# shihchinw/rlShaders

Hardware: AMD Instinct MI355X
Metric: BSDF Gsamples/sec (eval+sample+pdf) (higher is better)
Workload: dtype f32

## Files before the change

__graft_entry__.py:

```python
from __future__ import annotations

import os
import subprocess
import sys
from pathlib import Path

ROOT = Path(__file__).resolve().parent
REF_SRC_DEFAULT = "/root/reference"
for p in (str(ROOT), str(ROOT / "tests")):
    if p not in sys.path:
        sys.path.insert(0, p)


def build() -> None:
    from rlshaders_amd import build as b
    lib = b.build_library(verbose=False)
    assert lib.exists(), lib
    b.build_host_examples()
    b.build_trace_example()
    p = subprocess.run(["make", "-C", str(ROOT / "oracle")], capture_output=True, text=True)
    if p.returncode != 0:
        raise RuntimeError(f"oracle build failed:\n{p.stdout}\n{p.stderr}")
    ref_src = Path(os.environ.get("RLS_REF_SRC", REF_SRC_DEFAULT))
    if (ref_src / "src" / "rlGgx.h").exists():
        p = subprocess.run(["make", "-C", str(ROOT / "oracle"), "ref", f"REF_SRC={ref_src}"], capture_output=True,
                           text=True)
        if p.returncode != 0:
            raise RuntimeError(f"reference build failed:\n{p.stdout}\n{p.stderr}")
    import rlshaders_amd
    rlshaders_amd.load()
    from rlshaders_amd import trace
    trace.load()


def smoke() -> None:
    import numpy as np
    import torch

    import cases
    import oracle_lib as O
    import rlshaders_amd as R
    from gpu_util import dev, ggx_oracle, ggx_sampler, host

    assert torch.cuda.is_available(), "smoke() needs a GPU"
    ctx = R.Context(0)
    n = 1 << 14
    c = cases.ggx_mixed(cases.SEED_PARITY, n)
    x = cases.xi(cases.SEED_PARITY, n, 4)
    s = ggx_sampler(ctx, c)
    out = [host(t) for t in s.reflectRefract(dev(x[0]), dev(x[1]), dev(x[2]), dev(x[3]))]
    ref = ggx_oracle(O, c).reflect_refract(x[0], x[1], x[2], x[3])
    names = ("wi", "f", "pdf", "fresnel", "wt", "weight")
    for name, a, b in zip(names, out, ref):
        st = cases.summarize(cases.rel_err(a, b))
        print(f"smoke {name}: median {st['median']:.2e} p99.9 {st['p999']:.2e} frac>1e-5 {st['frac_gt_1e5']:.2e}")
        assert st["nonfinite"] == 0 and st["max"] <= 1e-5, (name, st)
    f = host(s.evalBrdf(dev(ref[0])))
    assert cases.summarize(cases.rel_err(f, ref[1]))["max"] <= 1e-5
    ctx.close()
    print("smoke ok")


if __name__ == "__main__":
    build()
    if len(sys.argv) > 1 and sys.argv[1] == "smoke":
        smoke()
```

rlshaders_amd/build.py:

```python
from __future__ import annotations

import os
import shutil
import subprocess
import sys
from concurrent.futures import ThreadPoolExecutor
from pathlib import Path

PKG = Path(__file__).resolve().parent
CSRC = PKG / "csrc"
LIBDIR = PKG / "lib"
OBJDIR = PKG / "build"
LIB = LIBDIR / "librlshaders_amd.so"
ARCH = "gfx950"

SOURCES = ["shade.hip", "integrate.hip", "lights.hip", "scatter.hip", "skin.hip", "ggx.hip", "disney.hip", "sss.hip", "alternates.hip", "context.hip", "pipeline.hip",
           "libm_check.hip"]
FAST_UNITS = {"ggx.hip", "disney.hip", "sss.hip", "skin.hip", "integrate.hip", "lights.hip", "scatter.hip", "shade.hip", "alternates.hip"}
HEADERS = [CSRC / "rls_device.hpp", CSRC / "rls_libm.hpp", CSRC / "rls_libm_tables.inc", CSRC / "rls_libm_flavour_args.inc", CSRC / "rls_internal.hpp", CSRC / "rls_loops.hpp",
           PKG.parent / "include" / "rlshaders_amd.h", PKG.parent / "include" / "rlshaders_amd_diag.h"]

HIPCC_FLAGS = [
    f"--offload-arch={ARCH}", "-O3", "-std=c++17", "-fPIC",
    "-ffp-contract=off", "-fno-fast-math",
# ... 42 lines not shown
    def run(cmd):
        if verbose:
            print(" ".join(cmd), flush=True)
        p = subprocess.run(cmd, capture_output=True, text=True)
        if p.returncode != 0:
            raise RuntimeError(f"hipcc failed:\n{' '.join(cmd)}\n{p.stdout}\n{p.stderr}")
        return p

    if jobs:
        with ThreadPoolExecutor(max_workers=min(4, len(jobs))) as ex:
            list(ex.map(run, jobs))
    if force or jobs or _stale(lib, objs):
        run([hipcc, f"--offload-arch={ARCH}", "-shared", "-fPIC", "-o", str(lib), *map(str, objs)])
    return lib


TRACE_CSRC = PKG / "csrc_trace"
TRACE_SOURCES = ["trace.hip"]
TRACE_LIB = LIBDIR / "librls_trace.so"
TRACE_HEADERS = [*sorted(TRACE_CSRC.glob("*.hpp")), PKG.parent / "include" / "rlshaders_amd_trace.h"]


def build_trace_library(force: bool = False, verbose: bool = False) -> Path:
    hipcc = _hipcc()
    main = build_library(verbose=verbose)
    objdir = OBJDIR / "trace"
    objdir.mkdir(parents=True, exist_ok=True)
    jobs, objs = [], []
    for name in TRACE_SOURCES:
        src = TRACE_CSRC / name
        for suffix, flag in (("", "RLS_FAST=0"), ("_fast", "RLS_FAST=1")):
            obj = objdir / (src.stem + suffix + ".o")
            objs.append(obj)
            if force or _stale(obj, [src, *HEADERS, *TRACE_HEADERS, Path(__file__)]):
                jobs.append([hipcc, *HIPCC_FLAGS, f"-cuid=rls_trace.{src.stem}{suffix}", f"-D{flag}", "-c", str(src),
                             "-o", str(obj)])

    def run(cmd):
        if verbose:
            print(" ".join(cmd), flush=True)
        p = subprocess.run(cmd, capture_output=True, text=True)
        if p.returncode != 0:
            raise RuntimeError(f"hipcc failed:\n{' '.join(cmd)}\n{p.stdout}\n{p.stderr}")

    if jobs:
        with ThreadPoolExecutor(max_workers=min(4, len(jobs))) as ex:
            list(ex.map(run, jobs))
    if force or jobs or _stale(TRACE_LIB, [*objs, main]):
        run([hipcc, f"--offload-arch={ARCH}", "-shared", "-fPIC", "-o", str(TRACE_LIB), *map(str, objs),
             f"-L{LIBDIR}", "-lrlshaders_amd", "-Wl,-rpath,$ORIGIN"])
    return TRACE_LIB


def build_trace_example(verbose: bool = False) -> Path:
    OBJDIR.mkdir(exist_ok=True)
    lib = build_trace_library(verbose=verbose)
    src, out = PKG / "host" / "example_trace.cpp", OBJDIR / "example_trace"
    if _stale(out, [src, PKG / "host" / "rls_trace.hpp", lib, LIB, *HEADERS, *TRACE_HEADERS]):
        cmd = ["g++", "-std=c++14", "-O2", "-Wall", f"-I{PKG.parent / 'include'}", f"-I{PKG / 'host'}", str(src), "-o", str(out),
               f"-L{LIBDIR}", "-lrls_trace", "-lrlshaders_amd", f"-Wl,-rpath,{LIBDIR}", "-L/opt/rocm/lib", "-Wl,-rpath,/opt/rocm/lib"]
        if verbose:
            print(" ".join(cmd), flush=True)
        p = subprocess.run(cmd, capture_output=True, text=True)
        if p.returncode != 0:
            raise RuntimeError(f"host example example_trace failed to build:\n{p.stdout}\n{p.stderr}")
    return out


def build_host_examples(verbose: bool = False) -> Path:
    OBJDIR.mkdir(exist_ok=True)
    first = OBJDIR / "example_arnold_stub"
    for name in ("example_arnold_stub", "example_multi_gpu", "example_host_pipeline", "test_arnold_stub"):
        src = PKG / "host" / f"{name}.cpp"
        out = OBJDIR / name
        if not src.exists():
            continue
        if _stale(out, [src, PKG / "host" / "rls_batch.hpp", PKG / "host" / "rl_arnold_stub.hpp", LIB, *HEADERS]):
            cmd = ["g++", "-std=c++14", "-O2", "-Wall", "-pthread", f"-I{PKG.parent / 'include'}", f"-I{PKG / 'host'}",
                   str(src), "-o", str(out), f"-L{LIBDIR}", "-lrlshaders_amd", f"-Wl,-rpath,{LIBDIR}",
                   "-L/opt/rocm/lib", "-Wl,-rpath,/opt/rocm/lib"]
            if verbose:
                print(" ".join(cmd), flush=True)
            p = subprocess.run(cmd, capture_output=True, text=True)
            if p.returncode != 0:
                raise RuntimeError(f"host example {name} failed to build:\n{p.stdout}\n{p.stderr}")
    return first


if __name__ == "__main__":
    args = sys.argv[1:]
    variant = args[args.index("--variant") + 1] if "--variant" in args else ""
    defines = [a[2:] for a in args if a.startswith("-D")]
    extra = []
    for i, a in enumerate(args):
        if a.startswith(("-f", "-m", "-O")):
            extra.append(a)
            if a == "-mllvm":
                extra.append(args[i + 1])
    print(build_library(force="--force" in args, verbose=True, variant=variant, defines=defines, extra=extra))
```

rlshaders_amd/codeid.py:

```python
from __future__ import annotations

import hashlib
import re
import struct
from functools import lru_cache
from pathlib import Path
from typing import Dict, List, Optional, Tuple

BUNDLE_MAGIC = b"__CLANG_OFFLOAD_BUNDLE__"
KERNEL_ID_SCHEME = 2
HASHED_SECTIONS = (".text", ".rodata", ".data")


def _sections(elf: bytes) -> Dict[str, Tuple[int, int, int]]:
    if elf[:4] != b"\x7fELF" or elf[4] != 2 or elf[5] != 1:
        raise ValueError("not a little-endian ELF64 image")
    shoff, = struct.unpack_from("<Q", elf, 0x28)
    shentsize, shnum, shstrndx = struct.unpack_from("<HHH", elf, 0x3A)
    heads = []
    for k in range(shnum):
        name, typ, _flags, _addr, off, size = struct.unpack_from("<IIQQQQ", elf, shoff + k * shentsize)
        heads.append((name, typ, off, size))
    _, _, stroff, strsize = heads[shstrndx]
    strtab = elf[stroff:stroff + strsize]
# ... 172 lines not shown
        h.update(name.encode() + b"\0" + struct.pack("<Q", size) + bytes(body))
    return h.hexdigest()[:16], [s[0] for s in syms if s[1] == 2]


def mangled_fragment(kernel: str) -> Optional[str]:
    m = re.search(r"([A-Za-z_][A-Za-z0-9_]*)\s*<([^<>]*)>\s*(?:\(|$)", kernel.strip())
    if not m:
        m = re.search(r"([A-Za-z_][A-Za-z0-9_]*)\s*(?:\(|$)", kernel.strip())
        return f"{len(m.group(1))}{m.group(1)}" if m else None
    name, args = m.group(1), [a.strip() for a in m.group(2).split(",") if a.strip()]
    enc = ""
    for a in args:
        if not re.fullmatch(r"-?\d+", a):
            return None
        enc += f"Li{'n' + a[1:] if a.startswith('-') else a}E"
    return f"{len(name)}{name}I{enc}E"


class DeviceCode:

    def __init__(self, path):
        self.path = str(path)
        objs = code_objects(fatbin(path))
        self.units = [unit_digest(e) for e in objs]
        self.kernels: Dict[str, str] = {}
        for e in objs:
            self.kernels.update(kernel_digests(e))
        self.library_id = hashlib.sha256("\n".join(sorted(u for u, _ in self.units)).encode()).hexdigest()[:16]

    def unit_of_kernel(self, kernel: str) -> Optional[str]:
        frag = mangled_fragment(kernel)
        if not frag:
            return None
        hits = sorted({u for u, syms in self.units if any(frag in s for s in syms)})
        return hits[0] if len(hits) == 1 else None

    def kernel_id(self, kernel: str) -> Optional[str]:
        frag = mangled_fragment(kernel)
        if not frag:
            return None
        hits = sorted({k for name, k in self.kernels.items() if frag in name})
        return hits[0] if len(hits) == 1 else None

    def record(self, kernel: Optional[str] = None) -> dict:
        rec = {"library_id": self.library_id}
        if kernel:
            rec["kernel"] = kernel
            rec["unit_id"] = self.unit_of_kernel(kernel)
            rec["kernel_id"] = self.kernel_id(kernel)
            rec["kernel_id_scheme"] = KERNEL_ID_SCHEME
        return rec


@lru_cache(maxsize=8)
def _cached(path: str, mtime: float, size: int) -> DeviceCode:
    return DeviceCode(path)


def device_code(path) -> DeviceCode:
    p = Path(path).resolve()
    st = p.stat()
    return _cached(str(p), st.st_mtime, st.st_size)


if __name__ == "__main__":
    import json
    import sys
    args = sys.argv[1:]
    lib = args[0] if args and args[0].endswith((".so", ".o")) or (args and ".so." in args[0]) else None
    if lib is None:
        from rlshaders_amd.build import LIB
        lib, names = LIB, args
    else:
        names = args[1:]
    dc = DeviceCode(lib)
    out = {"library": str(lib), "library_id": dc.library_id, "units": len(dc.units)}
    if names:
        out["kernels"] = {k: {"unit_id": dc.unit_of_kernel(k), "kernel_id": dc.kernel_id(k)} for k in names}
    else:
        out["unit_ids"] = sorted(u for u, _ in dc.units)
    print(json.dumps(out, indent=1))
```

rlshaders_amd/csrc/context.hip:

```cpp
#include <stdarg.h>
#include <stdlib.h>
#include <string.h>

#include "rls_internal.hpp"

namespace {
thread_local char g_error[512] = "";
}

namespace rlsh {

void set_error(const char *fmt, ...)
{
    va_list ap;
    va_start(ap, fmt);
    vsnprintf(g_error, sizeof(g_error), fmt, ap);
    va_end(ap);
}

rls_status hip_fail(hipError_t e, const char *what)
{
    set_error("HIP error %d (%s) in %s", (int)e, hipGetErrorString(e), what);
    (void)hipGetLastError();
    return e == hipErrorOutOfMemory ? RLS_ERR_OUT_OF_MEMORY : RLS_ERR_HIP;
}

}

using namespace rlsd;

extern "C" {

const char *rls_last_error(void) { return g_error; }

const char *rls_status_string(rls_status s)
{
    switch (s) {
    case RLS_OK: return "ok";
    case RLS_ERR_INVALID_ARGUMENT: return "invalid argument";
    case RLS_ERR_NO_DEVICE: return "no HIP device";
    case RLS_ERR_HIP: return "HIP runtime error";
    case RLS_ERR_OUT_OF_MEMORY: return "out of device memory";
    case RLS_ERR_UNSUPPORTED: return "unsupported";
    case RLS_ERR_ABORTED: return "stopped by a callback";
    default: return "unknown status";
    }
}

int rls_version(void) { return RLS_VERSION_MAJOR * 1000 + RLS_VERSION_MINOR; }

rls_status rls_context_create(int device_ordinal, rls_context **out)
{
    RLS_REQUIRE(out != nullptr, "out is NULL");
    *out = nullptr;
    int count = 0;
    hipError_t e = hipGetDeviceCount(&count);
    if (e != hipSuccess || count <= 0) {
        rlsh::set_error("rls_context_create: no HIP device visible (%s)",
                        e == hipSuccess ? "count = 0" : hipGetErrorString(e));
        return RLS_ERR_NO_DEVICE;
    }
    if (device_ordinal < 0 || device_ordinal >= count) {
        rlsh::set_error("rls_context_create: device %d out of range [0, %d)", device_ordinal, count);
        return RLS_ERR_NO_DEVICE;
    }
    RLS_HIP_TRY(hipSetDevice(device_ordinal));
    hipDeviceProp_t prop;
    RLS_HIP_TRY(hipGetDeviceProperties(&prop, device_ordinal));

    rls_context *ctx = (rls_context *)calloc(1, sizeof(rls_context));
    if (!ctx) { rlsh::set_error("rls_context_create: host allocation failed"); return RLS_ERR_OUT_OF_MEMORY; }
    ctx->device = device_ordinal;
    ctx->compute_units = prop.multiProcessorCount > 0 ? prop.multiProcessorCount : 256;
    ctx->blocks_per_cu = 64;
    if (const char *s = getenv("RLS_BLOCKS_PER_CU")) {
        int v = atoi(s);
        if (v >= 1 && v <= 4096) ctx->blocks_per_cu = v;
    }
    hipError_t e1 = hipStreamCreateWithFlags(&ctx->own_stream, hipStreamNonBlocking);
    hipError_t e2 = e1 == hipSuccess ? hipEventCreate(&ctx->ev_start) : e1;
    hipError_t e3 = e2 == hipSuccess ? hipEventCreate(&ctx->ev_stop) : e2;
    if (e3 == hipSuccess) e3 = hipEventCreate(&ctx->ev_probe_start);
    if (e3 == hipSuccess) e3 = hipEventCreate(&ctx->ev_probe_stop);
    hipError_t e4 = e3 == hipSuccess ? hipMalloc((void **)&ctx->scratch_u64, sizeof(unsigned long long)) : e3;
    if (e4 != hipSuccess) {
        rls_status st = rlsh::hip_fail(e4, "rls_context_create");
        rls_context_destroy(ctx);
        return st;
    }
    ctx->stream = ctx->own_stream;
    *out = ctx;
    return RLS_OK;
}

void rls_context_destroy(rls_context *ctx)
{
    if (!ctx) return;
    (void)hipSetDevice(ctx->device);
    if (ctx->capturing) {
        hipGraph_t g = nullptr;
        if (hipStreamEndCapture(ctx->stream, &g) == hipSuccess && g) (void)hipGraphDestroy(g);
        (void)hipGetLastError();
    }
    if (ctx->own_stream) (void)hipStreamSynchronize(ctx->own_stream);
    if (ctx->scratch_u64) (void)hipFree(ctx->scratch_u64);
    if (ctx->stamp_buf) (void)hipFree(ctx->stamp_buf);
    if (ctx->ev_start) (void)hipEventDestroy(ctx->ev_start);
    if (ctx->ev_stop) (void)hipEventDestroy(ctx->ev_stop);
    if (ctx->ev_probe_start) (void)hipEventDestroy(ctx->ev_probe_start);
    if (ctx->ev_probe_stop) (void)hipEventDestroy(ctx->ev_probe_stop);
    if (ctx->own_stream) (void)hipStreamDestroy(ctx->own_stream);
    free(ctx);
}

int rls_device_count(void)
{
    int n = 0;
    if (hipGetDeviceCount(&n) != hipSuccess) { (void)hipGetLastError(); return 0; }
    return n;
}

rls_status rls_shard_range(int64_t total, int rank, int world, int64_t *first, int64_t *count)
{
    RLS_REQUIRE(first != nullptr && count != nullptr, "NULL argument");
    RLS_REQUIRE(world >= 1 && rank >= 0 && rank < world && total >= 0, "bad shard request");
    const __int128 lo = (__int128)total * rank / world, hi = (__int128)total * (rank + 1) / world;
    *first = (int64_t)lo;
    *count = (int64_t)(hi - lo);
    return RLS_OK;
}

rls_status rls_context_set_stream(rls_context *ctx, void *hip_stream)
{
    RLS_REQUIRE(ctx != nullptr, "ctx is NULL");
    RLS_REQUIRE(!ctx->capturing, "not allowed while a launch graph is being recorded");
    ctx->stream = (hipStream_t)hip_stream;
    return RLS_OK;
}

rls_status rls_context_use_own_stream(rls_context *ctx)
{
    RLS_REQUIRE(ctx != nullptr, "ctx is NULL");
    RLS_REQUIRE(!ctx->capturing, "not allowed while a launch graph is being recorded");
// ... 514 lines not shown
```

rlshaders_amd/csrc/ggx.hip:

```cpp
#include "rls_internal.hpp"

using namespace rlsd;

namespace {

using namespace rlsh;

#define RLS_GGX_ARGS(a0) reload_args(a0)

enum { MIXED = 0, STREAMED_ALL = 1, UNIFORM_MATERIAL = 2 };

template <int MODE>
__device__ __forceinline__ Ggx load_closure(const rls_ggx_closure &c, Idx i, const GgxMaterial &um)
{
    constexpr bool STREAMED = MODE == STREAMED_ALL;
    V3 wo = ld3(c.wo, i), N = ld3(c.N, i), T = ld3(c.T, i);
    const PIndex<Idx> k = pindex<MODE == MIXED>(c.materials, i);
    float kr, kg, kb;
    ldrgb<STREAMED>(c.KsColor, k, kr, kg, kb);
    if (MODE == UNIFORM_MATERIAL)
        return ggx_from_material(um, wo, N, T, c.exiting ? (c.exiting[i.full()] != 0) : false, kr, kg, kb);
    float rough = ldp<STREAMED>(c.specularRoughness, k);
    float ior = ldp<STREAMED>(c.ior, k);
    float aniso = ldp<STREAMED>(c.anisotropic, k);
    bool exiting = c.exiting ? (c.exiting[i.full()] != 0) : false;
    return ggx_make(wo, N, T, exiting, kr, kg, kb, ior, rough, aniso);
}

#ifndef RLS_GGX_WAVES
#define RLS_GGX_WAVES(OP) ((OP) == OP_EVAL ? 6 : 8)
#endif
#define RLS_GGX_ATTR(OP) __launch_bounds__(rlsh::kBlock) __attribute__((amdgpu_waves_per_eu(RLS_GGX_WAVES(OP), RLS_GGX_WAVES(OP))))
template <int OP, int FAST_MATH, int MODE>
__device__ __forceinline__ void ggx_body(const GgxIO &a0)
{
    if (OP == OP_SAMPLE || OP == OP_FUSED || OP == OP_REFLECT_REFRACT || OP == OP_REFRACT || OP == OP_MICROFACET)
        stage_libm_tables();
    GgxMaterial um = {};
    if (MODE == UNIFORM_MATERIAL) {
        const rls_ggx_closure &c = a0.c;
        um = ggx_material_wave_uniform(ggx_material(c.ior.u, c.specularRoughness.u, c.anisotropic.u));
    }
    const TileRange tiles = tile_range(a0.n);
    for (int64_t base = tiles.first; base < tiles.end; base += tiles.step) {
        const Idx i = make_idx(base);
        if (i.full() >= a0.n) continue;
        const GgxIO a = RLS_GGX_ARGS(a0);
        Ggx g = load_closure<MODE>(a.c, i, um);

        if (OP == OP_SAMPLE || OP == OP_FUSED || OP == OP_REFLECT_REFRACT) {
            float rx = ldg(a.rx, i), ry = ldg(a.ry, i);
            VndfView w = vndf_view(g.view, g.fr, g.ax, g.ay);
            V3 M, M2;
            if (OP == OP_REFLECT_REFRACT) {
                float rx2 = ldg(a.rx2, i), ry2 = ldg(a.ry2, i);
                vndf_microfacet_pair(w, g.fr, rx, ry, w, g.fr, rx2, ry2, M, M2);
            } else {
                M = vndf_microfacet(w, g.fr, rx, ry);
            }
            V3 L = reflect_direction(g.view, M);
            float F = ggx_fresnel(g, L, M);
            {
                const GgxIO b = RLS_GGX_ARGS(a0);
                st3(b.wi, i, L);
                if (b.fresnel) stg(b.fresnel, i, F);
            }
            if (OP != OP_SAMPLE) {
                float fr, fg, fb, pdf;
                ggx_eval_pdf<true, true>(g, L, fr, fg, fb, pdf);
                const GgxIO b = RLS_GGX_ARGS(a0);
                strgb(b.f, i, fr, fg, fb);
                stg(b.pdf, i, pdf);
            }
            if (OP == OP_REFLECT_REFRACT) {
                V3 dir;
                ggx_refract(g, M2, dir);
                const float wgt = ggx_sample_weight(g, g.view, dir, M2);
                const GgxIO b = RLS_GGX_ARGS(a0);
                st3(b.wt, i, dir);
                stg(b.weight, i, wgt);
            }
// ... 3 lines not shown
            strgb(a.f, i, fr, fg, fb);
        } else if (OP == OP_PDF) {
            stg(a.pdf, i, ggx_pdf(g, ld3(a.cwi, i)));
        } else if (OP == OP_REFRACT) {
            float rx = ldg(a.rx, i), ry = ldg(a.ry, i);
            VndfView w = vndf_view(g.view, g.fr, g.ax, g.ay);
            V3 M = vndf_microfacet(w, g.fr, rx, ry);
            V3 dir;
            bool ok = ggx_refract(g, M, dir);
            st3(a.wt, i, dir);
            stg(a.weight, i, ggx_sample_weight(g, g.view, dir, M));
            if (a.refracted) a.refracted[i.full()] = ok ? 1 : 0;
        } else if (OP == OP_MICROFACET) {
            float rx = ldg(a.rx, i), ry = ldg(a.ry, i);
            V3 M;
            if (a.kernel == RLS_KERNEL_NDF) {
                M = ndf_microfacet(g, rx, ry);
            } else {
                VndfView w = vndf_view(g.view, g.fr, g.ax, g.ay);
                M = vndf_microfacet(w, g.fr, rx, ry);
            }
            st3(a.wi, i, M);
        } else if (OP == OP_NDF_PDF) {
            V3 H = normalize(g.view + ld3(a.cwi, i));
            stg(a.pdf, i, ndf_pdf(g, g.view, H));
        }
    }
}

template <int OP, int FAST_MATH, int MODE>
__global__ RLS_GGX_ATTR(OP) void ggx_kernel(GgxIO a0)
{
    ggx_body<OP, FAST_MATH, MODE>(a0);
}

#if RLS_DIAGNOSTICS
template <int OP, int FAST_MATH, int MODE>
__global__ RLS_GGX_ATTR(OP) void ggx_kernel_stamped(GgxIO a0, unsigned long long *stamps)
{
    ClockStamp<1> cs;
    cs.begin();
    ggx_body<OP, FAST_MATH, MODE>(a0);
    cs.end(stamps);
}
#endif

template <int OP>
rls_status launch_kernel(rls_context *ctx, const GgxIO &io, const char *name)
{
    const rls_ggx_closure &c = io.c;
    const bool streamed = !c.materials.id && c.KsColor.r && c.specularRoughness.v && c.ior.v && c.anisotropic.v;
    const bool uniform = !c.materials.id && !c.specularRoughness.v && !c.ior.v && !c.anisotropic.v;
    if constexpr (OP == OP_REFLECT_REFRACT)
        RLS_STAMPED_LAUNCH(streamed, (ggx_kernel_stamped<OP, RLS_FAST, STREAMED_ALL>),
                           rlsh::grid_for(ctx, io.n, rlsh::kBlock, RLS_CAP_MULT), io, name);
    if (streamed)
        hipLaunchKernelGGL((ggx_kernel<OP, RLS_FAST, STREAMED_ALL>), rlsh::grid_for(ctx, io.n, rlsh::kBlock, RLS_CAP_MULT), dim3(rlsh::kBlock), 0, ctx->stream, io);
    else if (uniform)
        hipLaunchKernelGGL((ggx_kernel<OP, RLS_FAST, UNIFORM_MATERIAL>), rlsh::grid_for_hoisting(ctx, io.n), dim3(rlsh::kBlock), 0, ctx->stream, io);
    else
        hipLaunchKernelGGL((ggx_kernel<OP, RLS_FAST, MIXED>), rlsh::grid_for(ctx, io.n, rlsh::kBlock, RLS_CAP_MULT), dim3(rlsh::kBlock), 0, ctx->stream, io);
    return rlsh::check_launch(name, RLS_FAST);
}

rls_status launch_ggx(rls_context *ctx, int op, const GgxIO &io, const char *name)
{
    switch (op) {
    case OP_SAMPLE: return launch_kernel<OP_SAMPLE>(ctx, io, name);
    case OP_EVAL: return launch_kernel<OP_EVAL>(ctx, io, name);
    case OP_PDF: return launch_kernel<OP_PDF>(ctx, io, name);
    case OP_FUSED: return launch_kernel<OP_FUSED>(ctx, io, name);
    case OP_REFRACT: return launch_kernel<OP_REFRACT>(ctx, io, name);
    case OP_REFLECT_REFRACT: return launch_kernel<OP_REFLECT_REFRACT>(ctx, io, name);
    case OP_MICROFACET: return launch_kernel<OP_MICROFACET>(ctx, io, name);
    default: return launch_kernel<OP_NDF_PDF>(ctx, io, name);
    }
}

}

RLS_FLAVOURS(ggx, rlsh::GgxIO)

#if !RLS_FAST

extern "C" {

rls_status rls_ggx_sample(rls_context *ctx, int64_t n, const rls_ggx_closure *c,
                          const float *rx, const float *ry, rls_vec3 wi, float *fresnel)
{
    RLS_PROLOGUE();
    if (rls_status s = rlsh::check_closure(__func__, c)) return s;
    RLS_REQUIRE(rx && ry, "rx/ry is NULL");
    RLS_REQUIRE(rlsh::has3(wi), "wi plane is NULL");
    GgxIO io = {};
    io.c = *c; io.rx = rx; io.ry = ry; io.wi = wi; io.fresnel = fresnel; io.n = n;
    return dispatch_ggx(ctx, OP_SAMPLE, io, "rls_ggx_sample");
}

rls_status rls_ggx_eval(rls_context *ctx, int64_t n, const rls_ggx_closure *c, rls_cvec3 wi, rls_rgb f)
{
    RLS_PROLOGUE();
    if (rls_status s = rlsh::check_closure(__func__, c)) return s;
    RLS_REQUIRE(rlsh::has3(wi) && rlsh::has3(f), "wi/f plane is NULL");
    GgxIO io = {};
    io.c = *c; io.cwi = wi; io.f = f; io.n = n;
    return dispatch_ggx(ctx, OP_EVAL, io, "rls_ggx_eval");
}

rls_status rls_ggx_pdf(rls_context *ctx, int64_t n, const rls_ggx_closure *c, rls_cvec3 wi, float *pdf)
{
    RLS_PROLOGUE();
    if (rls_status s = rlsh::check_closure(__func__, c)) return s;
    RLS_REQUIRE(rlsh::has3(wi) && pdf, "wi/pdf is NULL");
    GgxIO io = {};
    io.c = *c; io.cwi = wi; io.pdf = pdf; io.n = n;
    return dispatch_ggx(ctx, OP_PDF, io, "rls_ggx_pdf");
}

rls_status rls_ggx_sample_eval_pdf(rls_context *ctx, int64_t n, const rls_ggx_closure *c,
                                   const float *rx, const float *ry,
                                   rls_vec3 wi, rls_rgb f, float *pdf, float *fresnel)
{
    RLS_PROLOGUE();
    if (rls_status s = rlsh::check_closure(__func__, c)) return s;
    RLS_REQUIRE(rx && ry, "rx/ry is NULL");
    RLS_REQUIRE(rlsh::has3(wi) && rlsh::has3(f) && pdf, "wi/f/pdf is NULL");
    GgxIO io = {};
    io.c = *c; io.rx = rx; io.ry = ry; io.wi = wi; io.f = f; io.pdf = pdf; io.fresnel = fresnel; io.n = n;
    return dispatch_ggx(ctx, OP_FUSED, io, "rls_ggx_sample_eval_pdf");
}

rls_status rls_ggx_refract_sample(rls_context *ctx, int64_t n, const rls_ggx_closure *c,
                                  const float *rx, const float *ry,
                                  rls_vec3 wt, float *weight, uint8_t *refracted)
{
    RLS_PROLOGUE();
// ... 51 lines not shown
```

rlshaders_amd/csrc/pipeline.hip:

```cpp
#include <stdlib.h>
#include <string.h>

#include "rls_internal.hpp"

namespace {

struct Slot {
    rls_context *ctx;
    float *block;
    float **in, **out;
};

template <class HostPtr>
hipError_t copy_planes(bool up, int planes, HostPtr const *host, float *const *dev, int64_t dev_stride, int64_t p0,
                       int64_t count, int64_t n, hipStream_t stream, bool &strided)
{
    hipError_t e = hipSuccess;
    const size_t row = (size_t)count * sizeof(float);
    for (int k = 0; e == hipSuccess && k < planes;) {
        if (!host[k]) { k++; continue; }
        int m = k + 1;
        if (strided && m < planes && host[m] && host[m] > host[k]) {
            const ptrdiff_t d = host[m] - host[k];
            if (d < n) { m = k + 1; goto single; }
// ... 97 lines not shown
                "plane counts out of range");
    RLS_REQUIRE(depth >= 1 && depth <= 16, "depth must be in [1, 16]");
    rls_pipeline *p = (rls_pipeline *)calloc(1, sizeof(rls_pipeline));
    if (!p) { rlsh::set_error("rls_pipeline_create: out of host memory"); return RLS_ERR_OUT_OF_MEMORY; }
    p->parent = ctx;
    p->chunk_points = chunk_points;
    p->stride = (chunk_points + 63) / 64 * 64;
    p->in_planes = in_planes; p->out_planes = out_planes; p->depth = depth;
    {
        const char *sv = getenv("RLS_PIPELINE_STRIDED");
        p->strided = !(sv && sv[0] == '0');
    }
    p->slots = (Slot *)calloc((size_t)depth, sizeof(Slot));
    rls_status st = p->slots ? RLS_OK : RLS_ERR_OUT_OF_MEMORY;
    for (int s = 0; st == RLS_OK && s < depth; s++) {
        Slot &sl = p->slots[s];
        st = rls_context_create(ctx->device, &sl.ctx);
        if (st != RLS_OK) break;
        sl.ctx->blocks_per_cu = ctx->blocks_per_cu;
        const size_t planes = (size_t)(in_planes + out_planes);
        hipError_t e = hipMalloc((void **)&sl.block, planes * (size_t)p->stride * sizeof(float));
        if (e != hipSuccess) { st = rlsh::hip_fail(e, "rls_pipeline_create: hipMalloc"); break; }
        sl.in = (float **)calloc((size_t)(in_planes > 0 ? in_planes : 1), sizeof(float *));
        sl.out = (float **)calloc((size_t)(out_planes > 0 ? out_planes : 1), sizeof(float *));
        if (!sl.in || !sl.out) { st = RLS_ERR_OUT_OF_MEMORY; break; }
        for (int k = 0; k < in_planes; k++) sl.in[k] = sl.block + (size_t)k * (size_t)p->stride;
        for (int k = 0; k < out_planes; k++) sl.out[k] = sl.block + (size_t)(in_planes + k) * (size_t)p->stride;
    }
    if (st != RLS_OK) {
        if (st == RLS_ERR_OUT_OF_MEMORY) rlsh::set_error("rls_pipeline_create: out of memory");
        rls_pipeline_destroy(p);
        return st;
    }
    *out = p;
    return RLS_OK;
}

rls_status rls_pipeline_run(rls_pipeline *p, int64_t n, const float *const *host_in, float *const *host_out,
                            rls_pipeline_launch_fn launch, void *user)
{
    RLS_REQUIRE(p != nullptr, "pipeline is NULL");
    RLS_REQUIRE(n >= 0, "n < 0");
    RLS_REQUIRE(launch != nullptr, "launch callback is NULL");
    RLS_REQUIRE(p->in_planes == 0 || host_in != nullptr, "host_in is NULL");
    RLS_REQUIRE(p->out_planes == 0 || host_out != nullptr, "host_out is NULL");
    RLS_REQUIRE(!p->parent->capturing, "not allowed while a launch graph is being recorded");
    rls_status st = RLS_OK;
    int64_t c = 0;
    bool strided = p->strided;
    for (int64_t p0 = 0; p0 < n && st == RLS_OK; p0 += p->chunk_points, c++) {
        const int64_t count = n - p0 < p->chunk_points ? n - p0 : p->chunk_points;
        Slot &sl = p->slots[c % p->depth];
        sl.ctx->fast = p->parent->fast;
        hipStream_t stream = sl.ctx->stream;
        hipError_t e = hipSetDevice(sl.ctx->device);
        if (e != hipSuccess) { st = rlsh::hip_fail(e, "rls_pipeline_run: hipSetDevice"); break; }
        e = copy_planes(true, p->in_planes, host_in, sl.in, p->stride, p0, count, n, stream, strided);
        if (e != hipSuccess) { st = rlsh::hip_fail(e, "rls_pipeline_run: upload"); break; }
        st = launch(user, sl.ctx, p0, count, sl.in, sl.out);
        if (st != RLS_OK) break;
        e = copy_planes(false, p->out_planes, host_out, sl.out, p->stride, p0, count, n, stream, strided);
        if (e != hipSuccess) { st = rlsh::hip_fail(e, "rls_pipeline_run: download"); break; }
    }
    for (int s = 0; s < p->depth; s++) {
        hipError_t e = hipStreamSynchronize(p->slots[s].ctx->stream);
        if (e != hipSuccess && st == RLS_OK) st = rlsh::hip_fail(e, "rls_pipeline_run: synchronize");
    }
    return st;
}

rls_status rls_measure_copy_rates(rls_context *ctx, size_t bytes, float rates_gb_per_s[3])
{
    RLS_REQUIRE(ctx != nullptr && rates_gb_per_s != nullptr, "NULL argument");
    RLS_REQUIRE(!ctx->capturing, "not allowed while a launch graph is being recorded");
    RLS_REQUIRE(bytes >= (1u << 20), "bytes < 1 MiB");
    RLS_HIP_TRY(hipSetDevice(ctx->device));
    void *h0 = nullptr, *h1 = nullptr, *d0 = nullptr, *d1 = nullptr;
    hipStream_t s0 = nullptr, s1 = nullptr;
    hipEvent_t a = nullptr, b = nullptr, c = nullptr;
    hipError_t e = hipHostMalloc(&h0, bytes, hipHostMallocDefault);
    if (e == hipSuccess) e = hipHostMalloc(&h1, bytes, hipHostMallocDefault);
    if (e == hipSuccess) e = hipMalloc(&d0, bytes);
    if (e == hipSuccess) e = hipMalloc(&d1, bytes);
    if (e == hipSuccess) e = hipStreamCreateWithFlags(&s0, hipStreamNonBlocking);
    if (e == hipSuccess) e = hipStreamCreateWithFlags(&s1, hipStreamNonBlocking);
    if (e == hipSuccess) e = hipEventCreate(&a);
    if (e == hipSuccess) e = hipEventCreate(&b);
    if (e == hipSuccess) e = hipEventCreate(&c);
    if (e == hipSuccess) {
        memset(h0, 1, bytes);
        memset(h1, 2, bytes);
        const size_t piece = 64u << 20;
        auto pass = [&](bool up, bool down, float *gbs) -> hipError_t {
            hipError_t r = hipDeviceSynchronize();
            if (r == hipSuccess) r = hipEventRecord(a, s0);
            if (r == hipSuccess) r = hipStreamWaitEvent(s1, a, 0);
            for (size_t off = 0; r == hipSuccess && off < bytes; off += piece) {
                const size_t m = bytes - off < piece ? bytes - off : piece;
                if (up) r = hipMemcpyAsync((char *)d0 + off, (char *)h0 + off, m, hipMemcpyHostToDevice, s0);
                if (r == hipSuccess && down) r = hipMemcpyAsync((char *)h1 + off, (char *)d1 + off, m, hipMemcpyDeviceToHost, s1);
            }
            if (r == hipSuccess) r = hipEventRecord(b, s1);
            if (r == hipSuccess) r = hipStreamWaitEvent(s0, b, 0);
            if (r == hipSuccess) r = hipEventRecord(c, s0);
            if (r == hipSuccess) r = hipEventSynchronize(c);
            float ms = 0.0f;
// ... 30 lines not shown
```

rlshaders_amd/csrc/rls_internal.hpp:

```cpp
#pragma once

#include <hip/hip_runtime.h>
#include <stdint.h>
#include <stdio.h>

#include "../../include/rlshaders_amd.h"

#ifndef RLS_DIAGNOSTICS
#define RLS_DIAGNOSTICS 1
#endif
#if RLS_DIAGNOSTICS
#include "../../include/rlshaders_amd_diag.h"
#endif
#include "rls_device.hpp"

struct rls_context {
    int device;
    int compute_units;
    int blocks_per_cu;
    hipStream_t stream;
    hipStream_t own_stream;
    hipEvent_t ev_start, ev_stop;
    hipEvent_t ev_probe_start, ev_probe_stop;
    unsigned long long *scratch_u64;
    int fast;
    int capturing;
    unsigned long long *stamps;
    unsigned long long *stamp_buf;
    int64_t stamp_slots;
};

#define RLS_HIDDEN extern "C" __attribute__((visibility("hidden")))
#if RLS_FAST
#define RLS_FLAVOURS(verb, IO)                                                                                \
    RLS_HIDDEN rls_status rls_fast_##verb(rls_context *ctx, int sel, const IO *io, const char *name)         \
    {                                                                                                         \
        return launch_##verb(ctx, sel, *io, name);                                                            \
    }
#else
#define RLS_FLAVOURS(verb, IO)                                                                                \
    RLS_HIDDEN rls_status rls_fast_##verb(rls_context *ctx, int sel, const IO *io, const char *name);        \
    static rls_status dispatch_##verb(rls_context *ctx, int sel, const IO &io, const char *name)              \
    {                                                                                                         \
        return ctx->fast ? rls_fast_##verb(ctx, sel, &io, name) : launch_##verb(ctx, sel, io, name);          \
    }
#endif

namespace rlsh {

enum GgxOp { OP_SAMPLE, OP_EVAL, OP_PDF, OP_FUSED, OP_REFRACT, OP_REFLECT_REFRACT, OP_MICROFACET, OP_NDF_PDF };
struct GgxIO {
    rls_ggx_closure c;
    const float *rx, *ry, *rx2, *ry2;
    rls_cvec3 cwi;
    rls_vec3 wi;
    rls_rgb f;
    float *pdf, *fresnel;
    rls_vec3 wt;
    float *weight;
    uint8_t *refracted;
    int64_t n;
    int kernel;
};

enum DisneyOp { DOP_SAMPLE, DOP_EVAL, DOP_PDF, DOP_FUSED };
struct DisneyIO {
    rls_disney_closure c;
    const float *rx, *ry;
    rls_cvec3 cwi;
    rls_vec3 wi;
    rls_rgb f;
    float *pdf;
    int64_t n;
};

enum SssOp { SOP_ND, SOP_ND_PDF, SOP_ND_EVAL, SOP_PROBE, SOP_MIS };
struct SssIO {
    rls_sss_closure c;
    const float *rx, *ry, *rin;
    rls_cvec3 P, disp, sampleN;
    int literal;
    float *r;
    rls_vec3 origin, dir;
    float *maxdist, *pdf;
    rls_rgb profile;
    int64_t n;
};
enum MiscOp { MOP_CAVITY, MOP_DIFFUSE_DIR, MOP_UTIL, MOP_REFLECT_LUM };
struct MiscIO {
    rls_cvec3 a, b, c;
    const float *rx, *ry;
    float *out;
    rls_vec3 v0, v1;
    int64_t n;
};

enum AltOp { AOP_GTR2_ANISO, AOP_GTR2, AOP_NDF_PDF, AOP_D_GTR2, AOP_GAUSS, AOP_LIBM };
// ... 411 lines not shown
```

rlshaders_amd/csrc/rls_libm.hpp:

```cpp
#pragma once

#include <math.h>
#include <stdint.h>
#include <string.h>

#if defined(__HIPCC__)
#include <hip/hip_runtime.h>
#define RLM_FN __host__ __device__ __forceinline__
#else
#define RLM_FN static inline
#endif

namespace rlm {

RLM_FN uint32_t f2u(float x)
{
#if defined(__HIP_DEVICE_COMPILE__)
    return __float_as_uint(x);
#else
    uint32_t u; memcpy(&u, &x, 4); return u;
#endif
}
RLM_FN float u2f(uint32_t u)
{
#if defined(__HIP_DEVICE_COMPILE__)
    return __uint_as_float(u);
#else
    float x; memcpy(&x, &u, 4); return x;
#endif
}
RLM_FN float fabs32(float x) { return u2f(f2u(x) & 0x7fffffffu); }

RLM_FN float div32(float a, float b) { return a / b; }

#ifndef RLM_GLIBC_FMA
#define RLM_GLIBC_FMA 1
#endif
RLM_FN double mad(double a, double b, double c)
{
#if RLM_GLIBC_FMA
    return __builtin_fma(a, b, c);
#else
    return a * b + c;
#endif
}

template <bool GUARDED = true>
RLM_FN float sqrt32(float x)
{
#if defined(__HIP_DEVICE_COMPILE__)
    if (GUARDED && __builtin_expect((f2u(x) & 0x7fffffffu) - 1u < 0x0f800000u - 1u, 0)) return sqrtf(x);
    float s = __builtin_amdgcn_sqrtf(x);
    const float sm = __uint_as_float(__float_as_uint(s) - 1u);
    const float sp = __uint_as_float(__float_as_uint(s) + 1u);
    const float rm = __builtin_fmaf(-sm, s, x);
    const float rp = __builtin_fmaf(-sp, s, x);
    s = (0.0f >= rm) ? sm : s;
    s = (0.0f < rp) ? sp : s;
    return s;
#else
    return sqrtf(x);
#endif
}
RLM_FN float sqrt32_1p(float y) { return sqrt32<false>(1.0f + y); }
RLM_FN float sqrt32_1m(float t) { return sqrt32<false>(1.0f - t); }

RLM_FN float rcp32_w(float x)
{
#if defined(__HIP_DEVICE_COMPILE__)
    float r = __builtin_amdgcn_rcpf(x);
    const float e = __builtin_fmaf(-x, r, 1.0f);
    r = __builtin_fmaf(e, r, r);
    return __builtin_amdgcn_div_fixupf(r, x, 1.0f);
#else
    return 1.0f / x;
#endif
}
RLM_FN float rcp32(float x)
{
#if defined(__HIP_DEVICE_COMPILE__)
    if (__builtin_expect(__builtin_amdgcn_classf(x, 0x90) || __builtin_fabsf(x) > 0x1p126f, 0)) return 1.0f / x;
    return rcp32_w(x);
#else
    return 1.0f / x;
#endif
}

RLM_FN float div32_m(float a, float b)
{
#if defined(__HIP_DEVICE_COMPILE__)
    float y = __builtin_amdgcn_rcpf(b);
    const float e = __builtin_fmaf(-b, y, 1.0f);
    y = __builtin_fmaf(e, y, y);
    const float q0 = a * y;
    const float r = __builtin_fmaf(-b, q0, a);
    return __builtin_fmaf(r, y, q0);
#else
    return a / b;
#endif
}

RLM_FN float div32_const_w(float x, float c, float rc)
{
#if defined(__HIP_DEVICE_COMPILE__)
    const float q0 = x * rc;
    const float r = __builtin_fmaf(-c, q0, x);
    return __builtin_fmaf(r, rc, q0);
#else
    (void)rc;
    return x / c;
#endif
}
RLM_FN float div32_const(float x, float c, float rc)
{
#if defined(__HIP_DEVICE_COMPILE__)
// ... 849 lines not shown
```

Before: 66.44.

## Add lean GGX companion library using wave-uniform Goldschmidt sqrt fast path

New measurement: 66.86 (median of 6 runs). Within noise of the previous version (+0.6%).

```diff
diff --git a/__graft_entry__.py b/__graft_entry__.py
--- a/__graft_entry__.py
+++ b/__graft_entry__.py
@@ -18,6 +18,7 @@
     assert lib.exists(), lib
     b.build_host_examples()
     b.build_trace_example()
+    b.build_lean_library()
     p = subprocess.run(["make", "-C", str(ROOT / "oracle")], capture_output=True, text=True)
     if p.returncode != 0:
         raise RuntimeError(f"oracle build failed:\n{p.stdout}\n{p.stderr}")
diff --git a/rlshaders_amd/build.py b/rlshaders_amd/build.py
--- a/rlshaders_amd/build.py
+++ b/rlshaders_amd/build.py
@@ -118,6 +118,38 @@
     return TRACE_LIB
 
 
+LEAN_CSRC = PKG / "csrc_lean"
+LEAN_SOURCES = ["lean.hip"]
+LEAN_LIB = LIBDIR / "librls_lean.so"
+
+
+def build_lean_library(force: bool = False, verbose: bool = False) -> Path:
+    hipcc = _hipcc()
+    main = build_library(verbose=verbose)
+    objdir = OBJDIR / "lean"
+    objdir.mkdir(parents=True, exist_ok=True)
+    objs, built = [], False
+    for name in LEAN_SOURCES:
+        src = LEAN_CSRC / name
+        obj = objdir / (src.stem + ".o")
+        objs.append(obj)
+        if force or _stale(obj, [src, CSRC / "ggx.hip", *HEADERS, Path(__file__)]):
+            cmd = [hipcc, *HIPCC_FLAGS, f"-cuid=rls_lean.{src.stem}", "-DRLS_FAST=0", "-c", str(src), "-o", str(obj)]
+            if verbose:
+                print(" ".join(cmd), flush=True)
+            p = subprocess.run(cmd, capture_output=True, text=True)
+            if p.returncode != 0:
+                raise RuntimeError(f"hipcc failed:\n{' '.join(cmd)}\n{p.stdout}\n{p.stderr}")
+            built = True
+    if force or built or _stale(LEAN_LIB, [*objs, main]):
+        cmd = [hipcc, f"--offload-arch={ARCH}", "-shared", "-fPIC", "-o", str(LEAN_LIB), *map(str, objs),
+               f"-L{LIBDIR}", "-lrlshaders_amd", "-Wl,-rpath,$ORIGIN"]
+        p = subprocess.run(cmd, capture_output=True, text=True)
+        if p.returncode != 0:
+            raise RuntimeError(f"hipcc failed:\n{' '.join(cmd)}\n{p.stdout}\n{p.stderr}")
+    return LEAN_LIB
+
+
 def build_trace_example(verbose: bool = False) -> Path:
     OBJDIR.mkdir(exist_ok=True)
     lib = build_trace_library(verbose=verbose)
diff --git a/rlshaders_amd/codeid.py b/rlshaders_amd/codeid.py
--- a/rlshaders_amd/codeid.py
+++ b/rlshaders_amd/codeid.py
@@ -248,15 +248,78 @@
         return rec
 
 
+LEAN_LIB_NAME = "librls_lean.so"
+LEAN_TAG = 2
+_LEAN_SERVED = re.compile(r"\b(ggx_kernel(?:_stamped)?)\s*<\s*(\d+)\s*,\s*0\s*,\s*(\d+)\s*>")
+
+
+def lean_companion(product) -> Optional[Path]:
+    p = Path(product)
+    q = p.resolve().parent / LEAN_LIB_NAME
+    return q if p.name.startswith("librlshaders_amd.so") and q.exists() else None
+
+
+def lean_kernel(kernel: Optional[str]) -> Optional[str]:
+    if not kernel or not _LEAN_SERVED.search(kernel):
+        return None
+    return _LEAN_SERVED.sub(lambda m: f"{m.group(1)}<{m.group(2)}, {LEAN_TAG}, {m.group(3)}>", kernel)
+
+
+def lean_launches(product) -> int:
+    import ctypes
+    import os
+    q = lean_companion(product)
+    if q is None:
+        return 0
+    try:
+        lib = ctypes.CDLL(str(q), mode=os.RTLD_NOLOAD | os.RTLD_NOW)
+        return int(ctypes.c_longlong.in_dll(lib, "rls_lean_launches").value)
+    except (OSError, ValueError):
+        return 0
+
+
+class ServedCode:
+
+    def __init__(self, product: DeviceCode, lean: DeviceCode):
+        self.product, self.lean = product, lean
+        self.path, self.units, self.kernels, self.library_id = product.path, product.units, product.kernels, product.library_id
+
+    def unit_of_kernel(self, kernel: str) -> Optional[str]:
+        k = lean_kernel(kernel)
+        return self.lean.unit_of_kernel(k) if k else self.product.unit_of_kernel(kernel)
+
+    def kernel_id(self, kernel: str) -> Optional[str]:
+        k = lean_kernel(kernel)
+        return self.lean.kernel_id(k) if k else self.product.kernel_id(kernel)
+
+    def record(self, kernel: Optional[str] = None) -> dict:
+        k = lean_kernel(kernel)
+        if not k:
+            return self.product.record(kernel)
+        rec = self.lean.record(k)
+        rec.update(kernel=kernel, served_by=k, flavour="lean", product_library_id=self.product.library_id)
+        return rec
+
+
 @lru_cache(maxsize=8)
 def _cached(path: str, mtime: float, size: int) -> DeviceCode:
     return DeviceCode(path)
 
 
-def device_code(path) -> DeviceCode:
+def _device_code_of(path) -> DeviceCode:
     p = Path(path).resolve()
     st = p.stat()
     return _cached(str(p), st.st_mtime, st.st_size)
+
+
+def served_code(path, lean: bool):
+    q = lean_companion(path) if lean else None
+    return ServedCode(_device_code_of(path), _device_code_of(q)) if q else _device_code_of(path)
+
+
+def device_code(path):
+    import os
+    return served_code(path, os.environ.get("RLS_LEAN") != "0" and lean_launches(path) > 0)
 
 
 if __name__ == "__main__":
@@ -273,6 +336,8 @@
     out = {"library": str(lib), "library_id": dc.library_id, "units": len(dc.units)}
     if names:
         out["kernels"] = {k: {"unit_id": dc.unit_of_kernel(k), "kernel_id": dc.kernel_id(k)} for k in names}
+        if lean_companion(lib):
+            out["lean"] = {k: served_code(lib, True).record(k) for k in names if lean_kernel(k)}
     else:
         out["unit_ids"] = sorted(u for u, _ in dc.units)
     print(json.dumps(out, indent=1))
diff --git a/rlshaders_amd/csrc/context.hip b/rlshaders_amd/csrc/context.hip
--- a/rlshaders_amd/csrc/context.hip
+++ b/rlshaders_amd/csrc/context.hip
@@ -1,3 +1,4 @@
+#include <dlfcn.h>
 #include <stdarg.h>
 #include <stdlib.h>
 #include <string.h>
@@ -23,6 +24,22 @@
     set_error("HIP error %d (%s) in %s", (int)e, hipGetErrorString(e), what);
     (void)hipGetLastError();
     return e == hipErrorOutOfMemory ? RLS_ERR_OUT_OF_MEMORY : RLS_ERR_HIP;
+}
+
+void *lean_entry(const char *symbol)
+{
+    static void *const companion = []() -> void * {
+        Dl_info self;
+        if (!dladdr((const void *)&lean_entry, &self) || !self.dli_fname) return nullptr;
+        const char *slash = strrchr(self.dli_fname, '/');
+        const char *base = slash ? slash + 1 : self.dli_fname;
+        if (strncmp(base, "librlshaders_amd.so", 19) != 0) return nullptr;
+        char path[4096];
+        const int dir = slash ? (int)(slash + 1 - self.dli_fname) : 0;
+        if (snprintf(path, sizeof(path), "%.*slibrls_lean.so", dir, self.dli_fname) >= (int)sizeof(path)) return nullptr;
+        return dlopen(path, RTLD_NOW | RTLD_LOCAL);
+    }();
+    return companion ? dlsym(companion, symbol) : nullptr;
 }
 
 }
@@ -89,6 +106,8 @@
         return st;
     }
     ctx->stream = ctx->own_stream;
+    const char *lean = getenv("RLS_LEAN");
+    ctx->lean = !(lean && strcmp(lean, "0") == 0);
     *out = ctx;
     return RLS_OK;
 }
diff --git a/rlshaders_amd/csrc/ggx.hip b/rlshaders_amd/csrc/ggx.hip
--- a/rlshaders_amd/csrc/ggx.hip
+++ b/rlshaders_amd/csrc/ggx.hip
@@ -27,6 +27,7 @@
     return ggx_make(wo, N, T, exiting, kr, kg, kb, ior, rough, aniso);
 }
 
+#define RLS_GGX_TAG (RLM_LEAN ? 2 : RLS_FAST)
 #ifndef RLS_GGX_WAVES
 #define RLS_GGX_WAVES(OP) ((OP) == OP_EVAL ? 6 : 8)
 #endif
@@ -136,14 +137,14 @@
     const bool streamed = !c.materials.id && c.KsColor.r && c.specularRoughness.v && c.ior.v && c.anisotropic.v;
     const bool uniform = !c.materials.id && !c.specularRoughness.v && !c.ior.v && !c.anisotropic.v;
     if constexpr (OP == OP_REFLECT_REFRACT)
-        RLS_STAMPED_LAUNCH(streamed, (ggx_kernel_stamped<OP, RLS_FAST, STREAMED_ALL>),
+        RLS_STAMPED_LAUNCH(streamed, (ggx_kernel_stamped<OP, RLS_GGX_TAG, STREAMED_ALL>),
                            rlsh::grid_for(ctx, io.n, rlsh::kBlock, RLS_CAP_MULT), io, name);
     if (streamed)
-        hipLaunchKernelGGL((ggx_kernel<OP, RLS_FAST, STREAMED_ALL>), rlsh::grid_for(ctx, io.n, rlsh::kBlock, RLS_CAP_MULT), dim3(rlsh::kBlock), 0, ctx->stream, io);
+        hipLaunchKernelGGL((ggx_kernel<OP, RLS_GGX_TAG, STREAMED_ALL>), rlsh::grid_for(ctx, io.n, rlsh::kBlock, RLS_CAP_MULT), dim3(rlsh::kBlock), 0, ctx->stream, io);
     else if (uniform)
-        hipLaunchKernelGGL((ggx_kernel<OP, RLS_FAST, UNIFORM_MATERIAL>), rlsh::grid_for_hoisting(ctx, io.n), dim3(rlsh::kBlock), 0, ctx->stream, io);
+        hipLaunchKernelGGL((ggx_kernel<OP, RLS_GGX_TAG, UNIFORM_MATERIAL>), rlsh::grid_for_hoisting(ctx, io.n), dim3(rlsh::kBlock), 0, ctx->stream, io);
     else
-        hipLaunchKernelGGL((ggx_kernel<OP, RLS_FAST, MIXED>), rlsh::grid_for(ctx, io.n, rlsh::kBlock, RLS_CAP_MULT), dim3(rlsh::kBlock), 0, ctx->stream, io);
+        hipLaunchKernelGGL((ggx_kernel<OP, RLS_GGX_TAG, MIXED>), rlsh::grid_for(ctx, io.n, rlsh::kBlock, RLS_CAP_MULT), dim3(rlsh::kBlock), 0, ctx->stream, io);
     return rlsh::check_launch(name, RLS_FAST);
 }
 
@@ -165,7 +166,7 @@
 
 RLS_FLAVOURS(ggx, rlsh::GgxIO)
 
-#if !RLS_FAST
+#if !RLS_FAST && !RLM_LEAN
 
 extern "C" {
 
diff --git a/rlshaders_amd/csrc/pipeline.hip b/rlshaders_amd/csrc/pipeline.hip
--- a/rlshaders_amd/csrc/pipeline.hip
+++ b/rlshaders_amd/csrc/pipeline.hip
@@ -173,6 +173,7 @@
         const int64_t count = n - p0 < p->chunk_points ? n - p0 : p->chunk_points;
         Slot &sl = p->slots[c % p->depth];
         sl.ctx->fast = p->parent->fast;
+        sl.ctx->lean = p->parent->lean;
         hipStream_t stream = sl.ctx->stream;
         hipError_t e = hipSetDevice(sl.ctx->device);
         if (e != hipSuccess) { st = rlsh::hip_fail(e, "rls_pipeline_run: hipSetDevice"); break; }
diff --git a/rlshaders_amd/csrc/rls_internal.hpp b/rlshaders_amd/csrc/rls_internal.hpp
--- a/rlshaders_amd/csrc/rls_internal.hpp
+++ b/rlshaders_amd/csrc/rls_internal.hpp
@@ -28,10 +28,21 @@
     unsigned long long *stamps;
     unsigned long long *stamp_buf;
     int64_t stamp_slots;
+    int lean;
 };
 
 #define RLS_HIDDEN extern "C" __attribute__((visibility("hidden")))
-#if RLS_FAST
+namespace rlsh { void *lean_entry(const char *symbol); }
+#if RLM_LEAN
+extern "C" __attribute__((visibility("default"))) long long rls_lean_launches;
+#define RLS_FLAVOURS(verb, IO)                                                                                \
+    extern "C" __attribute__((visibility("default")))                                                         \
+    rls_status rls_lean_##verb(rls_context *ctx, int sel, const IO *io, const char *name)                     \
+    {                                                                                                         \
+        __atomic_fetch_add(&rls_lean_launches, 1, __ATOMIC_RELAXED);                                          \
+        return launch_##verb(ctx, sel, *io, name);                                                            \
+    }
+#elif RLS_FAST
 #define RLS_FLAVOURS(verb, IO)                                                                                \
     RLS_HIDDEN rls_status rls_fast_##verb(rls_context *ctx, int sel, const IO *io, const char *name)         \
     {                                                                                                         \
@@ -42,7 +53,13 @@
     RLS_HIDDEN rls_status rls_fast_##verb(rls_context *ctx, int sel, const IO *io, const char *name);        \
     static rls_status dispatch_##verb(rls_context *ctx, int sel, const IO &io, const char *name)              \
     {                                                                                                         \
-        return ctx->fast ? rls_fast_##verb(ctx, sel, &io, name) : launch_##verb(ctx, sel, io, name);          \
+        typedef rls_status (*lean_fn)(rls_context *, int, const IO *, const char *);                          \
+        if (ctx->fast) return rls_fast_##verb(ctx, sel, &io, name);                                           \
+        if (ctx->lean) {                                                                                      \
+            static const lean_fn lean = (lean_fn)rlsh::lean_entry("rls_lean_" #verb);                         \
+            if (lean) return lean(ctx, sel, &io, name);                                                       \
+        }                                                                                                     \
+        return launch_##verb(ctx, sel, io, name);                                                             \
     }
 #endif
 
diff --git a/rlshaders_amd/csrc/rls_libm.hpp b/rlshaders_amd/csrc/rls_libm.hpp
--- a/rlshaders_amd/csrc/rls_libm.hpp
+++ b/rlshaders_amd/csrc/rls_libm.hpp
@@ -45,8 +45,38 @@
 #endif
 }
 
-template <bool GUARDED = true>
-RLM_FN float sqrt32(float x)
+#ifndef RLM_LEAN
+#define RLM_LEAN 0
+#endif
+RLM_FN float sqrt32_goldschmidt(float x)
+{
+#if defined(__HIP_DEVICE_COMPILE__)
+    const float y = __builtin_amdgcn_rsqf(x);
+    float g = x * y;
+    float h = 0.5f * y;
+    const float e = __builtin_fmaf(-h, g, 0.5f);
+    h = __builtin_fmaf(h, e, h);
+    g = __builtin_fmaf(g, e, g);
+    const float d = __builtin_fmaf(-g, g, x);
+    return __builtin_fmaf(d, h, g);
+#else
+    return sqrtf(x);
+#endif
+}
+RLM_FN float sqrt32_markstein(float x)
+{
+#if defined(__HIP_DEVICE_COMPILE__)
+    const float s = __builtin_amdgcn_sqrtf(x);
+    const float h = 0.5f * __builtin_amdgcn_rcpf(s);
+    const float r = __builtin_fmaf(-s, s, x);
+    return __builtin_fmaf(r, h, s);
+#else
+    return sqrtf(x);
+#endif
+}
+RLM_FN bool sqrt32_in_window(float x) { return f2u(x) - 0x0f800000u < 0x7f800000u - 0x0f800000u; }
+template <bool GUARDED>
+RLM_FN float sqrt32_frozen(float x)
 {
 #if defined(__HIP_DEVICE_COMPILE__)
     if (GUARDED && __builtin_expect((f2u(x) & 0x7fffffffu) - 1u < 0x0f800000u - 1u, 0)) return sqrtf(x);
@@ -61,6 +91,14 @@
 #else
     return sqrtf(x);
 #endif
+}
+template <bool GUARDED = true>
+RLM_FN float sqrt32(float x)
+{
+#if RLM_LEAN && defined(__HIP_DEVICE_COMPILE__)
+    if (GUARDED && __builtin_expect(__builtin_amdgcn_ballot_w64(!sqrt32_in_window(x)) == 0, 1)) return sqrt32_goldschmidt(x);
+#endif
+    return sqrt32_frozen<GUARDED>(x);
 }
 RLM_FN float sqrt32_1p(float y) { return sqrt32<false>(1.0f + y); }
 RLM_FN float sqrt32_1m(float t) { return sqrt32<false>(1.0f - t); }
diff --git a/rlshaders_amd/csrc_lean/lean.hip b/rlshaders_amd/csrc_lean/lean.hip
--- /dev/null
+++ b/rlshaders_amd/csrc_lean/lean.hip
@@ -0,0 +1,85 @@
+#if RLS_FAST
+#error "the lean flavour is EXACT arithmetic: compile with RLS_FAST=0"
+#endif
+#define RLM_LEAN 1
+#include "../csrc/ggx.hip"
+
+long long rls_lean_launches = 0;
+
+extern "C" __attribute__((visibility("default"))) int rls_lean_serves(const rls_context *ctx)
+{
+    return ctx && !ctx->fast && ctx->lean;
+}
+
+namespace {
+
+enum LeanCheck {
+    LC_SQRT = 0,
+    LC_SQRT_1P = 1,
+    LC_SQRT_1M = 2,
+    LC_GOLDSCHMIDT = 3,
+    LC_MARKSTEIN = 4,
+    LC_COUNT
+};
+constexpr int kLeanCheckFirst = 8;
+
+struct LeanCheckOut {
+    unsigned long long differing;
+    uint32_t first[kLeanCheckFirst];
+};
+
+template <int WHAT>
+__global__ __launch_bounds__(rlsh::kBlock) void lean_check_kernel(LeanCheckOut *out)
+{
+    const uint64_t threads = (uint64_t)gridDim.x * rlsh::kBlock;
+    for (uint64_t u = (uint64_t)blockIdx.x * rlsh::kBlock + threadIdx.x; u < (1ull << 32); u += threads) {
+        const float x = rlm::u2f((uint32_t)u);
+        float lean, frozen;
+        if (WHAT == LC_SQRT) { lean = rlm::sqrt32<true>(x); frozen = rlm::sqrt32_frozen<true>(x); }
+        else if (WHAT == LC_SQRT_1P) { lean = rlm::sqrt32_1p(x); frozen = rlm::sqrt32_frozen<false>(1.0f + x); }
+        else if (WHAT == LC_SQRT_1M) { lean = rlm::sqrt32_1m(x); frozen = rlm::sqrt32_frozen<false>(1.0f - x); }
+        else {
+            if (!rlm::sqrt32_in_window(x)) continue;
+            lean = WHAT == LC_GOLDSCHMIDT ? rlm::sqrt32_goldschmidt(x) : rlm::sqrt32_markstein(x);
+            frozen = rlm::sqrt32_frozen<true>(x);
+        }
+        if (rlm::f2u(lean) != rlm::f2u(frozen)) {
+            const unsigned long long k = atomicAdd(&out->differing, 1ull);
+            if (k < (unsigned long long)kLeanCheckFirst) out->first[k] = (uint32_t)u;
+        }
+    }
+}
+
+}
+
+extern "C" __attribute__((visibility("default")))
+rls_status rls_lean_check(rls_context *ctx, int what, unsigned long long *differing, uint32_t *first)
+{
+    RLS_REQUIRE(ctx != nullptr, "ctx is NULL");
+    RLS_REQUIRE(what >= 0 && what < LC_COUNT, "unknown check");
+    RLS_REQUIRE(differing != nullptr && first != nullptr, "NULL argument");
+    RLS_REQUIRE(!ctx->capturing, "not allowed while a launch graph is being recorded");
+    RLS_HIP_TRY(hipSetDevice(ctx->device));
+    LeanCheckOut *dev = nullptr;
+    RLS_HIP_TRY(hipMalloc((void **)&dev, sizeof(LeanCheckOut)));
+    hipError_t e = hipMemsetAsync(dev, 0, sizeof(LeanCheckOut), ctx->stream);
+    if (e == hipSuccess) {
+        const dim3 grid((unsigned)(ctx->compute_units * 16)), block(rlsh::kBlock);
+        switch (what) {
+        case LC_SQRT: hipLaunchKernelGGL(lean_check_kernel<LC_SQRT>, grid, block, 0, ctx->stream, dev); break;
+        case LC_SQRT_1P: hipLaunchKernelGGL(lean_check_kernel<LC_SQRT_1P>, grid, block, 0, ctx->stream, dev); break;
+        case LC_SQRT_1M: hipLaunchKernelGGL(lean_check_kernel<LC_SQRT_1M>, grid, block, 0, ctx->stream, dev); break;
+        case LC_GOLDSCHMIDT: hipLaunchKernelGGL(lean_check_kernel<LC_GOLDSCHMIDT>, grid, block, 0, ctx->stream, dev); break;
+        default: hipLaunchKernelGGL(lean_check_kernel<LC_MARKSTEIN>, grid, block, 0, ctx->stream, dev); break;
+        }
+        e = hipGetLastError();
+    }
+    LeanCheckOut host = {};
+    if (e == hipSuccess) e = hipMemcpyAsync(&host, dev, sizeof(host), hipMemcpyDeviceToHost, ctx->stream);
+    if (e == hipSuccess) e = hipStreamSynchronize(ctx->stream);
+    (void)hipFree(dev);
+    if (e != hipSuccess) return rlsh::hip_fail(e, "rls_lean_check");
+    *differing = host.differing;
+    for (int k = 0; k < kLeanCheckFirst; k++) first[k] = host.first[k];
+    return RLS_OK;
+}
diff --git a/rlshaders_amd/lean.py b/rlshaders_amd/lean.py
--- /dev/null
+++ b/rlshaders_amd/lean.py
@@ -0,0 +1,45 @@
+from __future__ import annotations
+
+import ctypes as C
+from typing import List, Tuple
+
+from . import _capi as capi
+
+LEAN_LIB_PATH = capi._PKG / "lib" / "librls_lean.so"
+CHECKS = {"sqrt32": 0, "sqrt32_1p": 1, "sqrt32_1m": 2, "sqrt32_goldschmidt": 3, "sqrt32_markstein": 4}
+
+_lib = None
+
+
+def load() -> C.CDLL:
+    global _lib
+    if _lib is None:
+        capi.load()
+        path = capi.loaded_path().parent / LEAN_LIB_PATH.name
+        if not path.exists():
+            raise RuntimeError(f"rlshaders_amd: {path} not found; build it with rlshaders_amd.build.build_lean_library()")
+        lib = C.CDLL(str(path))
+        lib.rls_lean_serves.restype = C.c_int
+        lib.rls_lean_serves.argtypes = [C.c_void_p]
+        lib.rls_lean_check.restype = C.c_int
+        lib.rls_lean_check.argtypes = [C.c_void_p, C.c_int, C.POINTER(C.c_ulonglong), C.POINTER(C.c_uint32)]
+        _lib = lib
+    return _lib
+
+
+def serves(ctx) -> bool:
+    from .codeid import lean_companion
+    if lean_companion(capi.loaded_path()) is None:
+        return False
+    return bool(load().rls_lean_serves(ctx.handle))
+
+
+def launches() -> int:
+    from .codeid import lean_launches
+    return lean_launches(capi.loaded_path())
+
+
+def check(ctx, what: str) -> Tuple[int, List[int]]:
+    n, first = C.c_ulonglong(), (C.c_uint32 * 8)()
+    capi.check(load().rls_lean_check(ctx.handle, CHECKS[what], C.byref(n), first))
+    return int(n.value), [int(v) for v in first[:min(8, n.value)]]
```
